# Tamnemng/TAM-GCN

Measured on AMD Instinct MI355X. Metric: skeleton clips/sec (fwd+CE+bwd+grad all-reduce+SGD step), N-UCLA 20-joint x 64-frame, higher is better.
Workload: dtype f32 (exact fp32-input MFMA v_mfma_f32_16x16x4_f32 in every GEMM, forward and backward: the reference's arithmetic); 1 GPU; N-UCLA joint stream, 256 clips/GPU x (3,64,20,1), models.ctrgcn.Model fwd+CE+bwd+grad-allreduce+SGD step, train-mode BN; global_batch=256, streams=1, parallelism=dp1, launch=hipgraph, model_streams=0, rehearsal=False, allreduce=one flat bucket after backward

## Files before the change

### include/tamgcn.h

```cpp
#ifndef TAMGCN_H
#define TAMGCN_H

#ifdef __cplusplus
extern "C" {
#endif

#define TAMGCN_VERSION 401
#define TAMGCN_MAX_SUBSETS 3
#define TAMGCN_MAX_V 32

typedef struct tamgcn_src {
    const float* x1;
    const float* x2;
    const float* coef;
    int ctot;
    int coff;
    int act;
} tamgcn_src;

int         tamgcn_version(void);
const char* tamgcn_last_error(void);
const char* tamgcn_last_kernel(void);
int         tamgcn_get_split_mode(void);
int         tamgcn_set_split_mode(int mode);

int         tamgcn_ctrgc_lds_bytes(int S, int V, int R);

typedef struct tamgcn_conv_desc {
    tamgcn_src src;
    int N, K, T_in, V;
    const float* w;
    const float* bias;
    int M, KT, dil, stride, pad;
    int wmode;
    int up;
    float* y;
    int yctot, ycoff;
    int T_out;
    int T_y;
    int ostride;
    const float* add1;
    const float* add2;
    const float* bcast;
    float bcast_scale;
    const tamgcn_src* mask;
    const float* aux;
    const float* aux_center;
    int auxctot, auxcoff;
    float* stats_part;
    int stats_ctot, stats_coff;
    const float* post_coef;
    int post_ctot, post_act;
} tamgcn_conv_desc;

int tamgcn_conv_nparts(const tamgcn_conv_desc* d);
int tamgcn_conv(const tamgcn_conv_desc* d, void* stream);

int tamgcn_conv_signmask(const tamgcn_conv_desc* d, const unsigned char* bits, int bctot, int bcoff, void* stream);

typedef struct tamgcn_wgrad_desc {
    tamgcn_src gy;
    tamgcn_src src;
    int N, M, K, T_in, T_out, V, KT, dil, stride, pad;
    float* part;
    int nsplit;
} tamgcn_wgrad_desc;
int tamgcn_wgrad_max_split(const tamgcn_wgrad_desc* d);
int tamgcn_wgrad(const tamgcn_wgrad_desc* d, void* stream);

typedef struct tamgcn_conv_pair_desc {
    int N, T, V;
    int stride;
    tamgcn_src src;
    int K, M0, M1;
    const float* w0; const float* w1;
    const float* bias0; const float* bias1;
    float* y0; int yctot0, ycoff0;
    float* y1; int yctot1, ycoff1;
    float* stats_part0; int stats_ctot0, stats_coff0;
    float* stats_part1; int stats_ctot1, stats_coff1;
} tamgcn_conv_pair_desc;
int tamgcn_conv_pair(const tamgcn_conv_pair_desc* d, void* stream);

typedef struct tamgcn_wgrad_pair_desc {
    tamgcn_src gy0, gy1, src;
    int N, M0, M1, K, T, V;
    int stride;
    float* part;
    int nsplit;
} tamgcn_wgrad_pair_desc;
int tamgcn_wgrad_pair(const tamgcn_wgrad_pair_desc* d, void* stream);

typedef struct tamgcn_reduce_desc {
    const float* part; float* out;
    int nsplit, accumulate;
    long long stride_s, count;
    float scale;
} tamgcn_reduce_desc;
int tamgcn_reduce_multi(const tamgcn_reduce_desc* descs, int n, void* stream);

int tamgcn_reduce_sum(float* part, int nsplit, long long stride_s, long long count,
                      float scale, int accumulate, float* out, void* stream);

int tamgcn_bn_fwd_finalize(const float* part, int part_ctot, int part_coff, int nparts, double count,
                           const float* gamma, const float* beta,
                           float* running_mean, float* running_var, long long* num_batches_tracked,
                           float momentum, float eps, int training,
                           float* coef, float* save, int coef_ctot, int coef_coff, int C, void* stream);

int tamgcn_coef_diff(const float* coef_d, const float* coef_y, float* out, int C, int mode, void* stream);

int tamgcn_bn_bwd_finalize(const float* part, int part_ctot, int part_coff, int nparts, double count,
                           const float* gamma, const float* save, int save_ctot, int save_coff,
                           int training, float* dgamma, float* dbeta, float* dbias_conv,
                           float* coef, int coef_ctot, int coef_coff, int C, void* stream);

typedef struct tamgcn_bn_fwd_desc {
    const float* part; int part_ctot, part_coff, nparts; double count;
    const float* gamma; const float* beta; float* running_mean; float* running_var; long long* num_batches_tracked;
    float momentum, eps; int training;
    float* coef; float* save; int coef_ctot, coef_coff, C;
} tamgcn_bn_fwd_desc;
typedef struct tamgcn_bn_bwd_desc {
    const float* part; int part_ctot, part_coff, nparts; double count;
    const float* gamma; const float* save; int save_ctot, save_coff, training;
    float* dgamma; float* dbeta; float* dbias_conv; float* coef; int coef_ctot, coef_coff, C;
} tamgcn_bn_bwd_desc;
int tamgcn_bn_fwd_finalize_multi(const tamgcn_bn_fwd_desc* descs, int n, void* stream);
int tamgcn_bn_bwd_finalize_multi(const tamgcn_bn_bwd_desc* descs, int n, void* stream);

int tamgcn_tmean(const tamgcn_src* src, int N, int C, int T, int V, float* xbar, void* stream);

typedef struct tamgcn_ctrgc_desc {
    int N, Cin, Cout, S, R, T, V;
    tamgcn_src x;
    const float* pq;
    const float* w3;
    const float* b3;
    const float* w4;
    const float* b4;
    const float* A;
    const float* alpha;
    const float* E;
} tamgcn_ctrgc_desc;

int tamgcn_ctrgc_build_e(const tamgcn_ctrgc_desc* d, float* E, void* stream);

int tamgcn_ctrgc_fwd(const tamgcn_ctrgc_desc* d, float* y, float* stats_part, float* x3_out, void* stream);

int tamgcn_ctrgc_bwd_dx3(const tamgcn_ctrgc_desc* d, const tamgcn_src* dy,
                         float* dx3, float* db3_part, void* stream);

int tamgcn_ctrgc_bwd_de_acc(const tamgcn_ctrgc_desc* d, const tamgcn_src* dy, const float* x3,
                            float* dE, void* stream);
int tamgcn_ctrgc_bwd_de_tail(const tamgcn_ctrgc_desc* d, const float* dE,
                             float* dA_part, float* dw4_part, float* db4_part,
                             float* dalpha_part, float* dpq, int groups, void* stream);

int tamgcn_ctrgc_tiled_supported(int V);
int tamgcn_ctrgc_tiled_chunks(int V);
int tamgcn_ctrgc_tiled_build_e(const tamgcn_ctrgc_desc* d, float* E, void* stream);
int tamgcn_ctrgc_tiled_agg_fwd(const tamgcn_ctrgc_desc* d, const float* x3, const float* E, float* y, float* stats_part, void* stream);
int tamgcn_ctrgc_tiled_agg_bwd(const tamgcn_ctrgc_desc* d, const tamgcn_src* dy, const float* E, float* dx3, float* db3_part, void* stream);
int tamgcn_ctrgc_tiled_de_acc(const tamgcn_ctrgc_desc* d, const tamgcn_src* dy, const float* x3, float* dE, void* stream);
int tamgcn_ctrgc_tiled_de_tail(const tamgcn_ctrgc_desc* d, const float* dE, float* dA_part, float* dw4_part, float* db4_part,
                               float* dalpha_part, float* dpq, void* stream);

int tamgcn_vgen_supported(int V);
int tamgcn_vgen_lds_bytes(int S, int V, int R);
int tamgcn_vgen_build_e(const tamgcn_ctrgc_desc* d, float* E, void* stream);
int tamgcn_vgen_agg_fwd(const tamgcn_ctrgc_desc* d, const float* x3, const float* E, float* y, float* stats_part, void* stream);
int tamgcn_vgen_agg_bwd(const tamgcn_ctrgc_desc* d, const tamgcn_src* dy, const float* E, float* dx3, float* db3_part, void* stream);
int tamgcn_vgen_de_acc(const tamgcn_ctrgc_desc* d, const tamgcn_src* dy, const float* x3, float* dE, void* stream);
int tamgcn_vgen_de_tail(const tamgcn_ctrgc_desc* d, const float* dE, float* dA_part, float* dw4_part, float* db4_part,
                        float* dalpha_part, float* dpq, int groups, void* stream);

int tamgcn_ew_nparts(int N, int C, int T, int V);

int tamgcn_gcn_tail_fwd(const tamgcn_src* y, const tamgcn_src* o, const tamgcn_src* res,
                        int N, int C, int T, int V, float* g, void* stream);
int tamgcn_gcn_tail_bwd(const float* dg, const float* g, const tamgcn_src* o, const float* o_save,
                        int N, int C, int T, int V, float* dsum, float* doz, float* part, void* stream);
int tamgcn_gcn_tail_fwd_bits(const tamgcn_src* y, const tamgcn_src* o, const tamgcn_src* res,
// ... 241 lines not shown
```

### tam_gcn_amd/_lib.py

```python
import ctypes as C
import os

_HERE = os.path.dirname(os.path.abspath(__file__))
LIB_PATH = os.path.join(_HERE, 'libtamgcn.so')

c_float_p = C.c_void_p


class Src(C.Structure):
    _fields_ = [('x1', C.c_void_p), ('x2', C.c_void_p), ('coef', C.c_void_p),
                ('ctot', C.c_int), ('coff', C.c_int), ('act', C.c_int)]


class ConvDesc(C.Structure):
    _fields_ = [('src', Src),
                ('N', C.c_int), ('K', C.c_int), ('T_in', C.c_int), ('V', C.c_int),
                ('w', C.c_void_p), ('bias', C.c_void_p),
                ('M', C.c_int), ('KT', C.c_int), ('dil', C.c_int), ('stride', C.c_int), ('pad', C.c_int),
                ('wmode', C.c_int), ('up', C.c_int),
                ('y', C.c_void_p), ('yctot', C.c_int), ('ycoff', C.c_int),
                ('T_out', C.c_int), ('T_y', C.c_int), ('ostride', C.c_int),
                ('add1', C.c_void_p), ('add2', C.c_void_p), ('bcast', C.c_void_p), ('bcast_scale', C.c_float),
                ('mask', C.POINTER(Src)),
                ('aux', C.c_void_p), ('aux_center', C.c_void_p), ('auxctot', C.c_int), ('auxcoff', C.c_int),
# ... 64 lines not shown
                ('pq', C.c_void_p), ('w3', C.c_void_p), ('b3', C.c_void_p), ('w4', C.c_void_p),
                ('b4', C.c_void_p), ('A', C.c_void_p), ('alpha', C.c_void_p), ('E', C.c_void_p)]


class F2GcnDesc(C.Structure):
    _fields_ = [(k, C.c_int) for k in ('N', 'Cin', 'Cout', 'T', 'V', 'S', 'R', 'res_mode')] + \
               [(k, C.c_void_p) for k in ('x', 'w12', 'b12', 'w4', 'b4', 'A', 'alpha', 'w3', 'b3', 'sy', 'ty', 'wd', 'bd',
                                          'E', 'sum', 'diff', 'xpart')]


class F2GemmDesc(C.Structure):
    _fields_ = [(k, C.c_int) for k in ('N', 'K', 'M', 'T', 'V', 'mode', 'relu_rows')] + \
               [(k, C.c_void_p) for k in ('x', 'w', 'b', 'add', 'out')]


class F2TcnDesc(C.Structure):
    _fields_ = [(k, C.c_int) for k in ('N', 'Cin', 'Cout', 'T', 'V', 'stride', 'Cb', 'nb', 'ks', 'res_mode')] + \
               [('dil', C.c_int * 4), ('h', C.c_void_p), ('wt', C.c_void_p * 4), ('bt', C.c_void_p * 4)] + \
               [(k, C.c_void_p) for k in ('sp', 'tp', 'x', 'wr', 'br', 'out', 'xpart')]


class F2sGcnDesc(C.Structure):
    _fields_ = [(k, C.c_int) for k in ('N', 'Cin', 'Cout', 'T', 'V', 'K')] + \
               [(k, C.c_void_p) for k in ('x', 'Ae', 'wg', 'bg', 'h')]


class F2sTcnDesc(C.Structure):
    _fields_ = [(k, C.c_int) for k in ('N', 'Cin', 'Cout', 'T', 'V', 'KT', 'stride', 'res_mode')] + \
               [(k, C.c_void_p) for k in ('h', 'wt', 'bt', 'x', 'wr', 'br', 'out')]


class F2sTcnBwdDesc(C.Structure):
    _fields_ = [(k, C.c_int) for k in ('N', 'Cout', 'T', 'V', 'KT', 'stride')] + \
               [(k, C.c_void_p) for k in ('gout', 'out', 'h', 'wtb', 'dh')]


class F2sGcnBwdDesc(C.Structure):
    _fields_ = [(k, C.c_int) for k in ('N', 'Cin', 'Cout', 'T', 'V', 'K', 'stride', 'res_mode')] + \
               [(k, C.c_void_p) for k in ('dh', 'Ae', 'wgb', 'gout', 'out', 'wrb', 'dx')]


class OptimDesc(C.Structure):
    _fields_ = [('n', C.c_longlong),
                ('p', C.c_void_p), ('g', C.c_void_p), ('s0', C.c_void_p), ('s1', C.c_void_p),
                ('lr', C.c_void_p), ('step', C.c_void_p), ('scal', C.c_void_p),
                ('mode', C.c_int), ('nesterov', C.c_int),
                ('momentum', C.c_float), ('dampening', C.c_float), ('weight_decay', C.c_float), ('eps', C.c_float),
                ('beta1', C.c_double), ('beta2', C.c_double)]


class CeDesc(C.Structure):
    _fields_ = [('logits', C.c_void_p), ('labels', C.c_void_p), ('probs', C.c_void_p), ('weight', C.c_void_p),
                ('ignore_index', C.c_longlong), ('label_smoothing', C.c_double), ('reduction', C.c_int), ('N', C.c_int), ('K', C.c_int)]


class GradGuard(C.Structure):
    _fields_ = [('max_norm', C.c_float), ('skip_nonfinite', C.c_int), ('partial', C.c_void_p), ('n_partial', C.c_int),
                ('stat', C.c_void_p), ('skipped', C.c_void_p)]


_i, _p, _d, _f, _ll = C.c_int, C.c_void_p, C.c_double, C.c_float, C.c_longlong
_SP = C.POINTER(Src)
SIGNATURES = {
    'tamgcn_version': (_i, []),
    'tamgcn_last_error': (C.c_char_p, []),
    'tamgcn_last_kernel': (C.c_char_p, []),
    'tamgcn_ctrgc_lds_bytes': (_i, [_i, _i, _i]),
    'tamgcn_get_split_mode': (_i, []),
    'tamgcn_set_split_mode': (_i, [_i]),
    'tamgcn_conv_nparts': (_i, [C.POINTER(ConvDesc)]),
    'tamgcn_conv': (_i, [C.POINTER(ConvDesc), _p]),
    'tamgcn_wgrad_max_split': (_i, [C.POINTER(WgradDesc)]),
    'tamgcn_wgrad': (_i, [C.POINTER(WgradDesc), _p]),
    'tamgcn_conv_signmask': (_i, [C.POINTER(ConvDesc), _p, _i, _i, _p]),
    'tamgcn_conv_pair': (_i, [C.POINTER(ConvPairDesc), _p]),
    'tamgcn_wgrad_pair': (_i, [C.POINTER(WgradPairDesc), _p]),
    'tamgcn_stem_stats': (_i, [_p, _p, _p, _i, _i, _i, _i, _i, _p, _p]),
    'tamgcn_stem_apply': (_i, [_p, _p, _p, _i, _i, _i, _i, _i, _p, _p]),
    'tamgcn_head_pool_fwd': (_i, [_p, _i, _i, _i, _i, _i, _p, _p]),
    'tamgcn_head_pool_bwd': (_i, [_p, _i, _i, _i, _i, _i, _p, _p]),
    'tamgcn_head_fc_fwd': (_i, [_p, _p, _p, _i, _i, _i, _p, _p]),
    'tamgcn_head_fc_bwd': (_i, [_p, _p, _p, _i, _i, _i, _p, _p, _p, _p]),
    'tamgcn_reduce_multi': (_i, [C.POINTER(ReduceDesc), _i, _p]),
    'tamgcn_reduce_sum': (_i, [_p, _i, _ll, _ll, _f, _i, _p, _p]),
    'tamgcn_bn_fwd_finalize': (_i, [_p, _i, _i, _i, _d, _p, _p, _p, _p, _p, _f, _f, _i, _p, _p, _i, _i, _i, _p]),
    'tamgcn_bn_bwd_finalize': (_i, [_p, _i, _i, _i, _d, _p, _p, _i, _i, _i, _p, _p, _p, _p, _i, _i, _i, _p]),
    'tamgcn_bn_fwd_finalize_multi': (_i, [C.POINTER(BnFwdDesc), _i, _p]),
    'tamgcn_coef_diff': (_i, [_p, _p, _p, _i, _i, _p]),
    'tamgcn_bn_bwd_finalize_multi': (_i, [C.POINTER(BnBwdDesc), _i, _p]),
    'tamgcn_tmean': (_i, [_SP, _i, _i, _i, _i, _p, _p]),
    'tamgcn_ctrgc_build_e': (_i, [C.POINTER(CtrgcDesc), _p, _p]),
    'tamgcn_ctrgc_fwd': (_i, [C.POINTER(CtrgcDesc), _p, _p, _p, _p]),
    'tamgcn_ctrgc_bwd_dx3': (_i, [C.POINTER(CtrgcDesc), _SP, _p, _p, _p]),
    'tamgcn_ctrgc_bwd_de_acc': (_i, [C.POINTER(CtrgcDesc), _SP, _p, _p, _p]),
    'tamgcn_ctrgc_bwd_de_tail': (_i, [C.POINTER(CtrgcDesc), _p, _p, _p, _p, _p, _p, _i, _p]),
    'tamgcn_ctrgc_tiled_supported': (_i, [_i]),
    'tamgcn_ctrgc_tiled_chunks': (_i, [_i]),
    'tamgcn_ctrgc_tiled_build_e': (_i, [C.POINTER(CtrgcDesc), _p, _p]),
    'tamgcn_ctrgc_tiled_agg_fwd': (_i, [C.POINTER(CtrgcDesc), _p, _p, _p, _p, _p]),
    'tamgcn_ctrgc_tiled_agg_bwd': (_i, [C.POINTER(CtrgcDesc), _SP, _p, _p, _p, _p]),
    'tamgcn_ctrgc_tiled_de_acc': (_i, [C.POINTER(CtrgcDesc), _SP, _p, _p, _p]),
    'tamgcn_ctrgc_tiled_de_tail': (_i, [C.POINTER(CtrgcDesc), _p, _p, _p, _p, _p, _p, _p]),
    'tamgcn_vgen_supported': (_i, [_i]),
    'tamgcn_vgen_lds_bytes': (_i, [_i, _i, _i]),
    'tamgcn_vgen_build_e': (_i, [C.POINTER(CtrgcDesc), _p, _p]),
    'tamgcn_vgen_agg_fwd': (_i, [C.POINTER(CtrgcDesc), _p, _p, _p, _p, _p]),
    'tamgcn_vgen_agg_bwd': (_i, [C.POINTER(CtrgcDesc), _SP, _p, _p, _p, _p]),
    'tamgcn_vgen_de_acc': (_i, [C.POINTER(CtrgcDesc), _SP, _p, _p, _p]),
    'tamgcn_vgen_de_tail': (_i, [C.POINTER(CtrgcDesc), _p, _p, _p, _p, _p, _p, _i, _p]),
    'tamgcn_ew_nparts': (_i, [_i, _i, _i, _i]),
    'tamgcn_gcn_tail_fwd': (_i, [_SP, _SP, _SP, _i, _i, _i, _i, _p, _p]),
    'tamgcn_gcn_tail_bwd': (_i, [_p, _p, _SP, _p, _i, _i, _i, _i, _p, _p, _p, _p]),
    'tamgcn_gcn_tail_fwd_bits': (_i, [_SP, _SP, _SP, _i, _i, _i, _i, _p, _p, _p]),
    'tamgcn_gcn_tail_bwd_bits': (_i, [_p, _p, _SP, _p, _i, _i, _i, _i, _p, _p, _p, _p]),
    'tamgcn_gcn_mid_bwd': (_i, [_p, _p, _p, _p, _p, _p, _i, _i, _i, _i, _p, _p, _p, _p]),
    'tamgcn_tconv_supported': (_i, [_i, _i, _i, _i, C.POINTER(C.c_int), _i, _i]),
    'tamgcn_tconv_nparts': (_i, [C.POINTER(TconvDesc), _i]),
    'tamgcn_tconv_fwd': (_i, [C.POINTER(TconvDesc), _p]),
    'tamgcn_tconv_bwd': (_i, [C.POINTER(TconvDesc), _p]),
    'tamgcn_tconv_wgrad_max_split': (_i, [C.POINTER(TconvDesc)]),
    'tamgcn_tconv_wgrad': (_i, [C.POINTER(TconvDesc), _p]),
    'tamgcn_maxpool_fwd': (_i, [_SP, _i, _i, _i, _i, _i, _p, _i, _i, _i, _p, _p]),
    'tamgcn_maxpool_post_fwd': (_i, [_SP, _i, _i, _i, _i, _i, _p, _i, _i, _i, _p, _p, _i, _p]),
    'tamgcn_maxpool_bwd': (_i, [_SP, _SP, _p, _i, _i, _i, _i, _i, _i, _p, _i, _i, _p, _p]),
    'tamgcn_add_act_fwd': (_i, [_SP, _SP, _i, _i, _i, _i, _i, _p, _p, _p, _p]),
    'tamgcn_add_act_bwd': (_i, [_p, _p, _i, _p, _p, _p, _p, _i, _i, _i, _i, _p, _p, _p]),
    'tamgcn_add_act_fwd_bits': (_i, [_SP, _SP, _i, _i, _i, _i, _p, _p, _p, _p, _p]),
    'tamgcn_add_act_bwd_bits': (_i, [_p, _p, _p, _p, _p, _p, _i, _i, _i, _i, _p, _p, _p]),
    'tamgcn_apply': (_i, [_SP, _i, _i, _i, _i, _p, _i, _i, _p]),
    'tamgcn_score_fuse': (_i, [_p, _p, _i, _i, _i, _i, _p, _p, _p, _p, _p]),
    'tamgcn_ce_fwd': (_i, [_p, _p, _i, _i, _p, _p, _p]),
    'tamgcn_ce_bwd': (_i, [_p, _p, _i, _i, _p, _p]),
    'tamgcn_ce_opts_workspace_bytes': (_ll, [C.POINTER(CeDesc)]),
    'tamgcn_ce_opts_fwd': (_i, [C.POINTER(CeDesc), _p, _p, _p, _p]),
    'tamgcn_ce_opts_bwd_rows': (_i, [_p, _p, _i, _i, _p, _p]),
    'tamgcn_eval_accumulate': (_i, [_p, _p, _p, _i, _i, _i, _p, C.POINTER(C.c_int), _i, _ll, _ll, _p, _p, _p, _p, _p]),
    'tamgcn_score_sweep': (_i, [_p, _p, C.POINTER(C.c_float), _i, _i, _i, _i, _p, _p, _p]),
    'tamgcn_stream_derive': (_i, [_p, _i, _i, _i, _i, _i, _p, _i, _p, _p]),
    'tamgcn_feeder_transform': (_i, [_p, _p, _p, _p, _p, _i, _i, _i, _i, _i, _p, _p]),
    'tamgcn_feeder_draw': (_i, [_p, _ll, _p, _i, _p, _p, _p, _i, _i, _p, _p, _p, _p, _p]),
    'tamgcn_feeder_transform_indexed': (_i, [_p, _p, _ll, _p, _p, _p, _p, _i, _i, _i, _i, _i, _p, _p]),
    'tamgcn_clip_extent': (_i, [_p, _ll, _i, _i, _i, _i, _p, _p]),
    'tamgcn_clip_draw': (_i, [_p, _ll, _p, _i, _p, _p, _i, _i, _i, _i, _i, _i, _i, _p, _p, _p, _p, _p, _p, _p, _p, _p]),
    'tamgcn_clip_transform': (_i, [_p, _ll, _p, _p, _p, _p, _i, _i, _i, _i, _i, _i, _i, _p, _p]),
    'tamgcn_clip_crop_draw': (_i, [_p, _ll, _p, _i, _p, _p, _i, _d, _d, _i, _d, _p, _p, _p, _p, _p]),
    'tamgcn_clip_resize': (_i, [_p, _ll, _p, _p, _p, _i, _i, _i, _i, _i, _i, _p, _p]),
    'tamgcn_f2_e': (_i, [C.POINTER(F2GcnDesc), _p]),
    'tamgcn_f2_gcn': (_i, [C.POINTER(F2GcnDesc), _p]),
    'tamgcn_f2_gemm': (_i, [C.POINTER(F2GemmDesc), _p]),
    'tamgcn_f2_tcn': (_i, [C.POINTER(F2TcnDesc), _p]),
    'tamgcn_f2v_e': (_i, [C.POINTER(F2GcnDesc), _p]),
    'tamgcn_f2v_gcn': (_i, [C.POINTER(F2GcnDesc), _p]),
    'tamgcn_f2v_gemm': (_i, [C.POINTER(F2GemmDesc), _p]),
    'tamgcn_f2v_tcn': (_i, [C.POINTER(F2TcnDesc), _p]),
    'tamgcn_f2g_supported': (_i, [_i]),
    'tamgcn_f2g_lds_bytes': (_i, [_i, _i, _i, _i]),
    'tamgcn_f2g_e': (_i, [C.POINTER(F2GcnDesc), _p]),
    'tamgcn_f2g_gcn': (_i, [C.POINTER(F2GcnDesc), _p]),
    'tamgcn_f2g_gemm': (_i, [C.POINTER(F2GemmDesc), _p]),
    'tamgcn_f2g_tcn': (_i, [C.POINTER(F2TcnDesc), _p]),
    'tamgcn_f2_e_grouped': (_i, [C.POINTER(F2GcnDesc), _i, _p]),
    'tamgcn_f2_gcn_grouped': (_i, [C.POINTER(F2GcnDesc), _i, _p]),
    'tamgcn_f2_gemm_grouped': (_i, [C.POINTER(F2GemmDesc), _i, _p]),
    'tamgcn_f2_tcn_grouped': (_i, [C.POINTER(F2TcnDesc), _i, _p]),
    'tamgcn_f2v_e_grouped': (_i, [C.POINTER(F2GcnDesc), _i, _p]),
    'tamgcn_f2v_gcn_grouped': (_i, [C.POINTER(F2GcnDesc), _i, _p]),
# ... 60 lines not shown
```

### tam_gcn_amd/csrc/reduce.hip

```cpp
#include "common.h"

namespace {

__global__ __launch_bounds__(256) void reduce_sum_kernel(const float* part, int nsplit, long long stride_s, long long count,
                                                         float scale, int accumulate, float* out) {
    __shared__ double red[4][64];
    const int lane = threadIdx.x & 63, w = threadIdx.x >> 6;
    const long long e = (long long)blockIdx.x * 64 + lane;
    double s = 0.0;
    if (e < count)
        for (int k = w; k < nsplit; k += 4) s += (double)part[k * stride_s + e];
    red[w][lane] = s;
    __syncthreads();
    if (w == 0 && e < count) {
        double t = (red[0][lane] + red[1][lane]) + (red[2][lane] + red[3][lane]);
        float r = (float)(t * (double)scale);
        out[e] = accumulate ? out[e] + r : r;
    }
}

}

__global__ __launch_bounds__(256) void reduce_group_kernel(float* part, int nsplit, long long stride_s, long long count) {
    __shared__ double red[4][64];
    const int lane = threadIdx.x & 63, w = threadIdx.x >> 6;
    const long long e = (long long)blockIdx.x * 64 + lane;
    const int s0 = blockIdx.y * 64, s1 = min(nsplit, s0 + 64);
    double s = 0.0;
    if (e < count)
        for (int k = s0 + w; k < s1; k += 4) s += (double)part[k * stride_s + e];
    red[w][lane] = s;
    __syncthreads();
    if (w == 0 && e < count)
        part[(long long)s0 * stride_s + e] = (float)((red[0][lane] + red[1][lane]) + (red[2][lane] + red[3][lane]));
}

constexpr int RM_MAX = 24;
struct ReduceMulti { int n; tamgcn_reduce_desc d[RM_MAX]; };

__global__ __launch_bounds__(256) void reduce_multi_kernel(const ReduceMulti md) {
    __shared__ double red[4][64];
    const tamgcn_reduce_desc& d = md.d[blockIdx.y];
    const int lane = threadIdx.x & 63, w = threadIdx.x >> 6;
    const long long e = (long long)blockIdx.x * 64 + lane;
    if ((long long)blockIdx.x * 64 >= d.count) return;
    double s = 0.0;
    if (e < d.count) {
        const float* p = d.part + e;
        int k = w;
        for (; k + 28 < d.nsplit; k += 32) {
            float a[8];
#pragma unroll
            for (int i = 0; i < 8; ++i) a[i] = p[(long long)(k + 4 * i) * d.stride_s];
            s += ((double)a[0] + (double)a[1]) + ((double)a[2] + (double)a[3]);
            s += ((double)a[4] + (double)a[5]) + ((double)a[6] + (double)a[7]);
        }
        for (; k + 12 < d.nsplit; k += 16) {
            float a0 = p[(long long)k * d.stride_s], a1 = p[(long long)(k + 4) * d.stride_s];
            float a2 = p[(long long)(k + 8) * d.stride_s], a3 = p[(long long)(k + 12) * d.stride_s];
            s += ((double)a0 + (double)a1) + ((double)a2 + (double)a3);
        }
        for (; k < d.nsplit; k += 4) s += (double)p[(long long)k * d.stride_s];
    }
    red[w][lane] = s;
    __syncthreads();
    if (w == 0 && e < d.count) {
        double t = (red[0][lane] + red[1][lane]) + (red[2][lane] + red[3][lane]);
        float r = (float)(t * (double)d.scale);
        d.out[e] = d.accumulate ? d.out[e] + r : r;
    }
}

extern "C" int tamgcn_reduce_multi(const tamgcn_reduce_desc* descs, int n, void* stream) {
    TG_CHECK(descs && n > 0, "tamgcn_reduce_multi: bad args");
    for (int i0 = 0; i0 < n; i0 += RM_MAX) {
        ReduceMulti md;
        md.n = n - i0 < RM_MAX ? n - i0 : RM_MAX;
        long long maxc = 0;
        for (int i = 0; i < md.n; ++i) {
            md.d[i] = descs[i0 + i];
            TG_CHECK(md.d[i].part && md.d[i].out && md.d[i].nsplit > 0 && md.d[i].count > 0, "tamgcn_reduce_multi: bad descriptor %d", i0 + i);
            if (md.d[i].count > maxc) maxc = md.d[i].count;
        }
        hipLaunchKernelGGL(reduce_multi_kernel, dim3((unsigned)((maxc + 63) / 64), md.n), dim3(256), 0, (hipStream_t)stream, md);
    }
    tamgcn_note_kernel("reduce_multi_kernel");
    TG_LAUNCH_CHECK("tamgcn_reduce_multi");
    return 0;
}

extern "C" int tamgcn_reduce_sum(float* part, int nsplit, long long stride_s, long long count,
                                 float scale, int accumulate, float* out, void* stream) {
    TG_CHECK(part && out && nsplit > 0 && count > 0, "tamgcn_reduce_sum: bad args");
    long long blocks = (count + 63) / 64;
    if (nsplit > 128) {
        int groups = (nsplit + 63) / 64;
        TG_CHECK(groups <= 65535, "tamgcn_reduce_sum: too many splits");
        hipLaunchKernelGGL(reduce_group_kernel, dim3((unsigned)blocks, groups), dim3(256), 0, (hipStream_t)stream,
                           part, nsplit, stride_s, count);
        nsplit = groups;
        stride_s *= 64;
    }
    hipLaunchKernelGGL(reduce_sum_kernel, dim3((unsigned)blocks), dim3(256), 0, (hipStream_t)stream,
                       part, nsplit, stride_s, count, scale, accumulate, out);
    tamgcn_note_kernel("reduce_sum_kernel");
    TG_LAUNCH_CHECK("tamgcn_reduce_sum");
    return 0;
}
```

### tam_gcn_amd/distributed.py

```python
import torch
import torch.distributed as dist


class ParamArena:

    ALIGN = 16

    def __init__(self, model):
        seen, order, starts = set(), [], []
        for m in model.modules():
            if hasattr(m, '_arena_groups'):
                for grp in m._arena_groups():
                    first = True
                    for p in grp:
                        if p.requires_grad and id(p) not in seen:
                            seen.add(id(p)); order.append(p); starts.append(first)
                            first = False
        for p in model.parameters():
            if p.requires_grad and id(p) not in seen:
                seen.add(id(p)); order.append(p); starts.append(True)
        if not order:
            raise ValueError('no trainable parameters')
        dev, dt = order[0].device, order[0].dtype
        if any(p.device != dev or p.dtype != dt for p in order):
            raise ValueError('ParamArena needs all parameters on one device with one dtype')
        self.params, self.offsets = order, []
        off = 0
        for p, st in zip(order, starts):
            if st:
                off = (off + self.ALIGN - 1) // self.ALIGN * self.ALIGN
            self.offsets.append(off)
            off += p.numel()
        self.total = (off + self.ALIGN - 1) // self.ALIGN * self.ALIGN
        self.flat = torch.zeros(self.total, device=dev, dtype=dt)
        self.epoch = 0
        with torch.no_grad():
            for p, o in zip(order, self.offsets):
                v = self.flat[o:o + p.numel()].view(p.shape)
                v.copy_(p.data)
                p.data = v
                p._tamgcn_arena = self
        ptr = self.flat.untyped_storage().data_ptr()

        def clone_views(module, state, prefix, meta):
            for k, v in list(state.items()):
                if isinstance(v, torch.Tensor) and v.untyped_storage().data_ptr() == ptr:
                    state[k] = v.clone()
        self._hook = model._register_state_dict_hook(clone_views)

    def state_version(self):
        return (self.flat._version, self.epoch)

    def touch(self):
        self.epoch += 1

    def intact(self):
        base = self.flat.data_ptr()
        return all(p.data_ptr() == base + o * p.element_size() for p, o in zip(self.params, self.offsets))

    def grad_bucket(self):
        return FlatGradBucket(self.params, offsets=self.offsets, total=self.total)


class FlatGradBucket:

    def __init__(self, params, offsets=None, total=None):
        self.params = [p for p in params if p.requires_grad]
        if not self.params:
            raise ValueError('no trainable parameters')
        dev, dt = self.params[0].device, self.params[0].dtype
        if offsets is None:
            offsets, off = [], 0
            for p in self.params:
                offsets.append(off)
                off += p.numel()
            total = off
        self.offsets = list(offsets)
        self.flat = torch.zeros(total, device=dev, dtype=dt)
        self.views = [self.flat[o:o + p.numel()].view_as(p) for p, o in zip(self.params, self.offsets)]

    def zero(self):
        for p in self.params:
            p.grad = None

    def pack(self, accumulate=False, alpha=1.0):
        if accumulate:
            pairs = [(v, p.grad) for p, v in zip(self.params, self.views) if p.grad is not None and p.grad is not v]
            if pairs:
                torch._foreach_add_([v for v, _ in pairs], [g for _, g in pairs], alpha=alpha)
            for p, v in zip(self.params, self.views):
                p.grad = v
            return self.flat
        grads = [p.grad for p in self.params]
        if any(g is None for g in grads):
            self.flat.zero_()
            pairs = [(v, g) for v, g in zip(self.views, grads) if g is not None]
            if pairs:
                torch._foreach_copy_([v for v, _ in pairs], [g for _, g in pairs])
        else:
            torch._foreach_copy_(self.views, grads)
        for p, v in zip(self.params, self.views):
            p.grad = v
        return self.flat

    def all_reduce_mean(self, group=None, local_n=None, global_n=None):
        if dist.is_available() and dist.is_initialized() and dist.get_world_size(group) > 1:
            if local_n is not None:
                if not global_n:
                    raise ValueError('all_reduce_mean: local_n needs global_n')
                self.flat.mul_(float(local_n) / float(global_n))
                dist.all_reduce(self.flat, op=dist.ReduceOp.SUM, group=group)
            else:
                dist.all_reduce(self.flat, op=dist.ReduceOp.SUM, group=group)
                self.flat.div_(dist.get_world_size(group))
        return self.flat


class SegmentedReducer:

    def __init__(self, bucket, nseg=3, group=None, comm_stream=None):
        self.bucket, self.group = bucket, group
        n = len(bucket.params)
        nseg = max(1, min(int(nseg), n))
        total = sum(p.numel() for p in bucket.params)
        bounds, acc, target = [n], 0, total / nseg
        for i in range(n - 1, 0, -1):
            acc += bucket.params[i].numel()
            if acc >= target * len(bounds) and len(bounds) < nseg:
                bounds.append(i)
        bounds.append(0)
        self.ranges = [(bounds[k + 1], bounds[k]) for k in range(len(bounds) - 1)]
        self.seg_of = {}
        for k, (lo, hi) in enumerate(self.ranges):
            for i in range(lo, hi):
                self.seg_of[id(bucket.params[i])] = k
        ends = [bucket.offsets[hi] if hi < n else bucket.flat.numel() for _, hi in self.ranges]
        self.flat_ranges = [(bucket.offsets[lo], e) for (lo, _), e in zip(self.ranges, ends)]
        self.comm = comm_stream
        self._hooks = [p.register_post_accumulate_grad_hook(self._on_grad) for p in bucket.params]
        self.begin()

    def begin(self):
        self.left = [hi - lo for lo, hi in self.ranges]
        self.sent = [False] * len(self.ranges)
        self.scale = None

    def _distributed(self):
        return dist.is_available() and dist.is_initialized() and dist.get_world_size(self.group) > 1

    def _pack(self, k):
        lo, hi = self.ranges[k]
        b = self.bucket
        pairs = [(b.views[i], b.params[i].grad) for i in range(lo, hi)]
        f0, f1 = self.flat_ranges[k]
        if any(g is None for _, g in pairs):
            b.flat[f0:f1].zero_()
        live = [(v, g) for v, g in pairs if g is not None and g.data_ptr() != v.data_ptr()]
        if live:
            torch._foreach_copy_([v for v, _ in live], [g for _, g in live])
        for i in range(lo, hi):
            b.params[i].grad = b.views[i]

    def _send(self, k, local_n=None, global_n=None):
        self._pack(k)
        self.sent[k] = True
        if not self._distributed():
            return
        f0, f1 = self.flat_ranges[k]
        seg = self.bucket.flat[f0:f1]
        if self.comm is not None and seg.is_cuda:
            self.comm.wait_stream(torch.cuda.current_stream(seg.device))
            with torch.cuda.stream(self.comm):
                dist.all_reduce(seg, op=dist.ReduceOp.SUM, group=self.group)
        else:
            dist.all_reduce(seg, op=dist.ReduceOp.SUM, group=self.group)

    def _on_grad(self, p):
        k = self.seg_of.get(id(p))
        if k is None or self.sent[k]:
            return
        self.left[k] -= 1
        if self.left[k] == 0:
            self._send(k)

    def finish(self):
        for k in range(len(self.ranges)):
            if not self.sent[k]:
                self._send(k)
        flat = self.bucket.flat
        if self.comm is not None and flat.is_cuda:
            torch.cuda.current_stream(flat.device).wait_stream(self.comm)
        if self._distributed():
            flat.div_(dist.get_world_size(self.group))
        return flat

    def remove(self):
        for h in self._hooks:
            h.remove()
        self._hooks = []


def broadcast_state(module, src=0, group=None, arena=None):
    if not (dist.is_available() and dist.is_initialized()) or dist.get_world_size(group) == 1:
        return
    rest = list(module.parameters()) + list(module.buffers())
    if arena is not None:
        if not arena.intact():
            raise ValueError('broadcast_state: the ParamArena no longer backs the parameters')
        dist.broadcast(arena.flat, src=src, group=group)
        arena.touch()
        inside = {id(p) for p in arena.params}
        rest = [t for t in rest if id(t) not in inside]
    by_type = {}
    for t in rest:
        by_type.setdefault((t.dtype, t.device), []).append(t.data)
    with torch.no_grad():
        for ts in by_type.values():
            flat = torch.cat([t.reshape(-1) for t in ts])
            dist.broadcast(flat, src=src, group=group)
            off = 0
            for t in ts:
                t.copy_(flat[off:off + t.numel()].view_as(t))
                off += t.numel()


# ... 39 lines not shown
```

### tam_gcn_amd/ops.py

```python
import ctypes as C
import os
import threading

import torch

from . import _lib
from ._lib import Src, ConvDesc, WgradDesc, CtrgcDesc, ReduceDesc, TconvDesc, TCONV_MAXB

RELU = 1


def _stream():
    return C.c_void_p(torch.cuda.current_stream().cuda_stream)


def _ptr(t):
    if t is None:
        return None
    if not (t.is_cuda and t.is_contiguous()):
        raise RuntimeError('tam_gcn_amd: expected a contiguous HIP (cuda) tensor; there is no CPU path')
    if t.dtype not in (torch.float32, torch.int64, torch.int32, torch.float64, torch.uint8):
        raise RuntimeError(f'tam_gcn_amd: unsupported dtype {t.dtype}')
    return t.data_ptr()


class S:
    __slots__ = ('x1', 'x2', 'coef', 'coff', 'act', 'ctot')

    def __init__(self, x1, x2=None, coef=None, coff=0, act=0):
        self.x1, self.x2, self.coef, self.coff, self.act = x1, x2, coef, coff, act
        self.ctot = x1.shape[1]
        if x2 is not None and x2.shape != x1.shape:
            raise RuntimeError('tam_gcn_amd: x1/x2 geometry mismatch')
        if coef is not None and tuple(coef.shape) != (3, self.ctot):
            raise RuntimeError(f'tam_gcn_amd: coef shape {tuple(coef.shape)} != (3,{self.ctot})')

    def c(self):
        return Src(_ptr(self.x1), _ptr(self.x2), _ptr(self.coef), self.ctot, self.coff, self.act)


def _lib_():
    return _lib.load()


CHUNK_ELEMS = int(os.environ.get("TAMGCN_CHUNK_ELEMS", str(2 ** 32 - 1)))


def n_chunks(N, per_clip):
    c = max(1, CHUNK_ELEMS // max(1, per_clip))
    return [(i, min(N, i + c)) for i in range(0, N, c)]


def _slice_src(src, n0, n1):
    return S(src.x1[n0:n1], None if src.x2 is None else src.x2[n0:n1], src.coef, src.coff, src.act)


SLACK = 4


def empty(*shape, like):
    n = 1
    for d_ in shape:
        n *= d_
    return torch.empty(n + SLACK, device=like.device, dtype=torch.float32)[:n].view(shape)


def empty_like(t):
    return empty(*t.shape, like=t)


def zeros_like(t):
    return empty(*t.shape, like=t).zero_()


def with_slack(t):
    if t is None or t.shape[-1] % 4 == 0:
        return t
    st = t.untyped_storage()
    if st.nbytes() - (t.storage_offset() + t.numel()) * t.element_size() >= 4 * SLACK:
        return t
    out = empty(*t.shape, like=t)
    out.copy_(t)
    return out


def conv(src, K, w, bias, M, KT=1, dil=1, stride=1, pad=0, wmode=0, up=1,
         y=None, ycoff=0, T_out=None, T_y=None, ostride=1, add1=None, add2=None,
         bcast=None, bcast_scale=0.0, mask=None, aux=None, aux_center=None, auxcoff=0, stats=False,
         post_coef=None, post_act=0, sign=None, sign_coff=0):
# ... 226 lines not shown
    return part


def tconv_wgrad_pays(V, Cb, stride):
    if V > 32:
        return True
    if V % 4:
        return Cb >= 32 or stride > 1
    return Cb >= 64


def tconv_wgrad(gy, src, Cb, KT, dils, stride):
    N, _, T_in, V = src.x1.shape
    T_out = gy.x1.shape[2]
    if V % 4:
        gy = S(with_slack(gy.x1), with_slack(gy.x2), gy.coef, gy.coff, gy.act)
        src = S(with_slack(src.x1), None, src.coef, src.coff, src.act)
    nb = len(dils)
    d = TconvDesc()
    d.src = gy.c()
    d.N, d.T_in, d.T_out, d.V, d.Cb, d.nb, d.KT, d.stride = N, T_in, T_out, V, Cb, nb, KT, stride
    for b, dl in enumerate(dils):
        d.dil[b] = int(dl)
    mc = src.c()
    d.mask = C.pointer(mc)
    lib = _lib_()
    mx = lib.tamgcn_tconv_wgrad_max_split(C.byref(d))
    if mx <= 0:
        raise RuntimeError('tamgcn_tconv_wgrad: no tiling for this shape')
    blocks = nb * (1 if Cb == 16 else (Cb // 32) ** 2)
    nsplit = max(1, min(mx, WGRAD_BLOCKS * 2 // blocks))
    part = empty(nsplit, nb, Cb, Cb, KT, like=gy.x1)
    d.y, d.yctot, d.ycoff = _ptr(part), nsplit, 0
    _lib.check(lib.tamgcn_tconv_wgrad(C.byref(d), _stream()), 'tamgcn_tconv_wgrad')
    return reduce_sum(part, nsplit, chunks=[(Cb, Cb, KT, 1)] * nb)


WGRAD_BLOCKS = int(os.environ.get('TAMGCN_WGRAD_BLOCKS', '512'))


def wgrad(gy, src, M, K, KT=1, dil=1, stride=1, pad=0, rows=None):
    N, _, T_out, V = gy.x1.shape
    T_in = src.x1.shape[2]
    per_clip = max(gy.x1.shape[1] * T_out * V, src.x1.shape[1] * T_in * V)
    chunks = n_chunks(N, per_clip) if N * per_clip > CHUNK_ELEMS else [(0, N)]
    lib = _lib_()
    descs = []
    for n0, n1 in chunks:
        g_, s_ = (gy, src) if len(chunks) == 1 else (_slice_src(gy, n0, n1), _slice_src(src, n0, n1))
        descs.append((_wgrad_desc(g_, s_, M, K, KT, dil, stride, pad), g_, s_))
    splits = [_wgrad_splits(d, len(chunks)) for d, _, _ in descs]
    nsplit = sum(splits)
    part = empty(nsplit, M, K, KT, like=gy.x1)
    off = 0
    for (d, _, _), ns in zip(descs, splits):
        d.part, d.nsplit = part.data_ptr() + 4 * off * M * K * KT, ns
        _lib.check(lib.tamgcn_wgrad(C.byref(d), _stream()), 'tamgcn_wgrad')
        off += ns
    if rows is not None:
        return reduce_sum(part, nsplit, chunks=[(m, K, KT, 1) for m in rows])
    if nsplit == 1:
        return part.view(M, K, KT, 1)
    return reduce_sum(part, nsplit).view(M, K, KT, 1)


class ReduceBatch:
    _tls = threading.local()

    @staticmethod
    def active():
        return getattr(ReduceBatch._tls, 'active', None)

    def __enter__(self):
        self.items, self.prev = [], ReduceBatch.active()
        ReduceBatch._tls.active = self
        return self

    def __exit__(self, *exc):
        ReduceBatch._tls.active = self.prev
        if self.items and exc[0] is None:
            arr = (ReduceDesc * len(self.items))()
            for i, (part, nsplit, stride, off, count, scale, acc, out) in enumerate(self.items):
                arr[i] = ReduceDesc(part.data_ptr() + 4 * off, _ptr(out), nsplit, int(acc), stride, count, scale)
            _lib.check(_lib_().tamgcn_reduce_multi(arr, len(self.items), _stream()), 'tamgcn_reduce_multi')
        self.items = []
        return False


def reduce_sum(part, nsplit, scale=1.0, out=None, accumulate=False, chunks=None, immediate=False):
    count = part.numel() // nsplit
    if chunks is not None:
        outs, off = [], 0
        flat = part.view(nsplit, count)
        for shp in chunks:
            n = 1
            for d_ in shp:
                n *= d_
            o = torch.empty(shp, device=part.device, dtype=torch.float32)
            _reduce_piece(flat, nsplit, count, off, n, scale, o)
            outs.append(o)
            off += n
        assert off == count, 'reduce_sum: chunk shapes do not cover the slab'
        return outs
    if out is None:
        out = torch.empty(part.shape[1:], device=part.device, dtype=torch.float32)
    _reduce_piece(part, nsplit, count, 0, count, scale, out, accumulate, immediate)
    return out


def _reduce_piece(part, nsplit, stride, off, count, scale, out, accumulate=False, immediate=False):
    rb = None if immediate else ReduceBatch.active()
    if rb is not None:
        rb.items.append((part, nsplit, stride, off, count, scale, accumulate, out))
        return
    src = C.c_void_p(part.data_ptr() + 4 * off)
    if nsplit > 128:
        tmp = part.view(nsplit, stride)[:, off:off + count].contiguous()
        _lib.check(_lib_().tamgcn_reduce_sum(_ptr(tmp), nsplit, count, count, scale, int(accumulate), _ptr(out), _stream()),
                   'tamgcn_reduce_sum')
        return
    _lib.check(_lib_().tamgcn_reduce_sum(src, nsplit, stride, count, scale, int(accumulate), _ptr(out), _stream()),
               'tamgcn_reduce_sum')


def coef_diff(coef_d, coef_y, mode):
    out = torch.empty_like(coef_y)
    _lib.check(_lib_().tamgcn_coef_diff(_ptr(coef_d), _ptr(coef_y), _ptr(out), coef_y.shape[1], mode, _stream()), 'tamgcn_coef_diff')
    return out


def bn_fwd_finalize(part, part_coff, count, gamma, beta, rmean, rvar, nbt, momentum, eps, training,
                    coef, save, coff, C_):
    lib = _lib_()
    if part is not None:
        pctot, nparts = part.shape[1], part.shape[2]
    else:
        pctot, nparts = 0, 0
    _lib.check(lib.tamgcn_bn_fwd_finalize(_ptr(part), pctot, part_coff, nparts, float(count),
                                          _ptr(gamma), _ptr(beta), _ptr(rmean), _ptr(rvar), _ptr(nbt),
                                          momentum, eps, int(training), _ptr(coef), _ptr(save),
                                          coef.shape[1], coff, C_, _stream()), 'tamgcn_bn_fwd_finalize')


class BNBatch:

    def __init__(self):
        self.f, self.b, self.keep = [], [], []

    def fwd(self, part, part_coff, count, gamma, beta, rmean, rvar, nbt, momentum, eps, training, coef, save, coff, C_):
        d = _lib.BnFwdDesc()
        d.part = _ptr(part)
        d.part_ctot, d.nparts = (part.shape[1], part.shape[2]) if part is not None else (0, 0)
        d.part_coff, d.count = part_coff, float(count)
        d.gamma, d.beta, d.running_mean, d.running_var, d.num_batches_tracked = _ptr(gamma), _ptr(beta), _ptr(rmean), _ptr(rvar), _ptr(nbt)
        d.momentum, d.eps, d.training = momentum, eps, int(training)
        d.coef, d.save, d.coef_ctot, d.coef_coff, d.C = _ptr(coef), _ptr(save), coef.shape[1], coff, C_
        self.f.append(d)
        self.keep += [part, coef, save]

    def bwd(self, part, part_coff, count, gamma, save, save_coff, training, dgamma, dbeta, dbias, coef, coff, C_):
        d = _lib.BnBwdDesc()
        d.part, d.part_ctot, d.part_coff, d.nparts, d.count = _ptr(part), part.shape[1], part_coff, part.shape[2], float(count)
        d.gamma, d.save, d.save_ctot, d.save_coff, d.training = _ptr(gamma), _ptr(save), save.shape[1], save_coff, int(training)
        d.dgamma, d.dbeta, d.dbias_conv = _ptr(dgamma), _ptr(dbeta), _ptr(dbias)
        d.coef, d.coef_ctot, d.coef_coff, d.C = _ptr(coef), coef.shape[1], coff, C_
        self.b.append(d)
        self.keep += [part, save, coef, dgamma, dbeta, dbias]
# ... 761 lines not shown
```

Baseline: 9404 clips/s.

## Defer weight-gradient split reductions to one batched flush into the flat grad bucket

Split-K weight-gradient reductions issued during backward are now queued on the host instead of launched one batch at a time. They are flushed at pack time as a few large queued-reduce kernels, and each destination is retargeted so the reduction writes straight into the flat all-reduce bucket view. This is meant to cut many small reduce launches and the extra foreach copy of gradients into the bucket. It also adds a deeper-unrolled reduction loop. In exchange, partial slabs stay alive longer (up to a memory cap), the host keeps queue state that must stay consistent with hipgraph capture, and a poison mode exists for debugging.

Result: no change. 9444 clips/s (median of 6 runs) (+0.4%).

```diff
diff --git a/include/tamgcn.h b/include/tamgcn.h
--- a/include/tamgcn.h
+++ b/include/tamgcn.h
@@ -99,6 +99,12 @@
 } tamgcn_reduce_desc;
 int tamgcn_reduce_multi(const tamgcn_reduce_desc* descs, int n, void* stream);
 
+int tamgcn_reduce_defer(const tamgcn_reduce_desc* descs, int n);
+int tamgcn_reduce_flush(void* stream);
+int tamgcn_reduce_pending(void);
+int tamgcn_reduce_retarget(const void* old_out, void* new_out);
+int tamgcn_reduce_discard(void);
+
 int tamgcn_reduce_sum(float* part, int nsplit, long long stride_s, long long count,
                       float scale, int accumulate, float* out, void* stream);
 
diff --git a/tam_gcn_amd/_defer.py b/tam_gcn_amd/_defer.py
--- /dev/null
+++ b/tam_gcn_amd/_defer.py
@@ -0,0 +1,157 @@
+import ctypes as C
+import math
+import os
+
+import torch
+
+from . import _lib
+
+_armed = {}
+_owner = {}
+_held = {}
+_held_bytes = {}
+_dest = {}
+
+
+def _load():
+    return _lib.load()
+
+
+def _guard(idx):
+    return torch.cuda.device(idx)
+
+
+def _stream_of(idx):
+    return torch.cuda.current_stream(idx)
+
+
+def mode():
+    v = os.environ.get('TAMGCN_DEFER_REDUCE', '1').strip().lower()
+    if v in ('0', 'off', 'false', 'no'):
+        return 'off'
+    return 'poison' if v == 'poison' else 'on'
+
+
+def max_bytes():
+    return int(os.environ.get('TAMGCN_DEFER_MAX_BYTES', str(2 << 30)))
+
+
+def _is_gpu(device):
+    return device.type == 'cuda'
+
+
+def _index(device):
+    return device.index if device.index is not None else torch.cuda.current_device()
+
+
+def armed(device):
+    return bool(_armed) and _is_gpu(device) and _index(device) in _armed
+
+
+def _clear(idx):
+    _held.pop(idx, None)
+    _held_bytes.pop(idx, None)
+    _dest.pop(idx, None)
+
+
+def _drop(idx):
+    _owner.pop(idx, None)
+    if _armed.pop(idx, None) is not None or _held.get(idx):
+        with _guard(idx):
+            _load().tamgcn_reduce_discard()
+    _clear(idx)
+
+
+def arm(device, owner=None):
+    if not _is_gpu(device):
+        return False
+    idx = _index(device)
+    _drop(idx)
+    m = mode()
+    if m == 'off':
+        return False
+    _armed[idx] = m
+    _owner[idx] = owner
+    return True
+
+
+def abandon(device, owner):
+    if _armed and _is_gpu(device):
+        idx = _index(device)
+        if idx in _armed and _owner.get(idx) == owner:
+            _drop(idx)
+
+
+def defer(device, arr, items):
+    idx = _index(device)
+    held = _held.setdefault(idx, {})
+    new = {id(it[0]): it[0] for it in items if id(it[0]) not in held}
+    nbytes = sum(p.numel() * p.element_size() for p in new.values())
+    if _held_bytes.get(idx, 0) + nbytes > max_bytes():
+        return False
+    with _guard(idx):
+        _lib.check(_load().tamgcn_reduce_defer(arr, len(items)), 'tamgcn_reduce_defer')
+    held.update(new)
+    _held_bytes[idx] = _held_bytes.get(idx, 0) + nbytes
+    dest = _dest.setdefault(idx, {})
+    poison = _armed.get(idx) == 'poison'
+    for it in items:
+        count, acc, out = it[4], it[6], it[7]
+        if not acc:
+            dest[out.data_ptr()] = count
+            if poison:
+                out.fill_(math.nan)
+    return True
+
+
+def retarget(device, pairs):
+    idx = _index(device)
+    dest = _dest.get(idx)
+    if not dest:
+        return pairs
+    rest = []
+    with _guard(idx):
+        lib = _load()
+        for v, g in pairs:
+            ptr = g.data_ptr()
+            if (dest.get(ptr) == g.numel() == v.numel() and g.dtype == v.dtype == torch.float32 and g.is_contiguous()
+                    and v.is_contiguous() and lib.tamgcn_reduce_retarget(ptr, v.data_ptr()) == 1):
+                del dest[ptr]
+                continue
+            rest.append((v, g))
+    return rest
+
+
+def flush(device):
+    if not _is_gpu(device):
+        return 0
+    idx = _index(device)
+    held = _held.get(idx)
+    if not held:
+        _clear(idx)
+        return 0
+    with _guard(idx):
+        st = _stream_of(idx)
+        for part in held.values():
+            part.record_stream(st)
+        rc = _load().tamgcn_reduce_flush(C.c_void_p(st.cuda_stream))
+    _clear(idx)
+    if rc < 0:
+        _lib.check(rc, 'tamgcn_reduce_flush')
+    return rc
+
+
+def disarm(device):
+    if not _is_gpu(device) or not (_armed or _held):
+        return 0
+    n = flush(device)
+    _armed.pop(_index(device), None)
+    _owner.pop(_index(device), None)
+    return n
+
+
+def pending(device):
+    if not _is_gpu(device):
+        return 0
+    with _guard(_index(device)):
+        return _load().tamgcn_reduce_pending()
diff --git a/tam_gcn_amd/_lib.py b/tam_gcn_amd/_lib.py
--- a/tam_gcn_amd/_lib.py
+++ b/tam_gcn_amd/_lib.py
@@ -170,6 +170,11 @@
     'tamgcn_head_fc_fwd': (_i, [_p, _p, _p, _i, _i, _i, _p, _p]),
     'tamgcn_head_fc_bwd': (_i, [_p, _p, _p, _i, _i, _i, _p, _p, _p, _p]),
     'tamgcn_reduce_multi': (_i, [C.POINTER(ReduceDesc), _i, _p]),
+    'tamgcn_reduce_defer': (_i, [C.POINTER(ReduceDesc), _i]),
+    'tamgcn_reduce_flush': (_i, [_p]),
+    'tamgcn_reduce_pending': (_i, []),
+    'tamgcn_reduce_retarget': (_i, [_p, _p]),
+    'tamgcn_reduce_discard': (_i, []),
     'tamgcn_reduce_sum': (_i, [_p, _i, _ll, _ll, _f, _i, _p, _p]),
     'tamgcn_bn_fwd_finalize': (_i, [_p, _i, _i, _i, _d, _p, _p, _p, _p, _p, _f, _f, _i, _p, _p, _i, _i, _i, _p]),
     'tamgcn_bn_bwd_finalize': (_i, [_p, _i, _i, _i, _d, _p, _p, _i, _i, _i, _p, _p, _p, _p, _i, _i, _i, _p]),
diff --git a/tam_gcn_amd/csrc/reduce.hip b/tam_gcn_amd/csrc/reduce.hip
--- a/tam_gcn_amd/csrc/reduce.hip
+++ b/tam_gcn_amd/csrc/reduce.hip
@@ -1,4 +1,7 @@
 #include "common.h"
+#include <mutex>
+#include <unordered_map>
+#include <vector>
 
 namespace {
 
@@ -38,16 +41,24 @@
 constexpr int RM_MAX = 24;
 struct ReduceMulti { int n; tamgcn_reduce_desc d[RM_MAX]; };
 
-__global__ __launch_bounds__(256) void reduce_multi_kernel(const ReduceMulti md) {
-    __shared__ double red[4][64];
-    const tamgcn_reduce_desc& d = md.d[blockIdx.y];
-    const int lane = threadIdx.x & 63, w = threadIdx.x >> 6;
-    const long long e = (long long)blockIdx.x * 64 + lane;
-    if ((long long)blockIdx.x * 64 >= d.count) return;
+template <int DEPTH>
+__device__ __forceinline__ void reduce_slabs(const tamgcn_reduce_desc& d, long long e, int lane, int w, double (*red)[64]) {
     double s = 0.0;
     if (e < d.count) {
         const float* p = d.part + e;
         int k = w;
+        if (DEPTH > 1) {
+            for (; k + 32 * DEPTH - 4 < d.nsplit; k += 32 * DEPTH) {
+                float a[8 * DEPTH];
+#pragma unroll
+                for (int i = 0; i < 8 * DEPTH; ++i) a[i] = p[(long long)(k + 4 * i) * d.stride_s];
+#pragma unroll
+                for (int j = 0; j < DEPTH; ++j) {
+                    s += ((double)a[8 * j + 0] + (double)a[8 * j + 1]) + ((double)a[8 * j + 2] + (double)a[8 * j + 3]);
+                    s += ((double)a[8 * j + 4] + (double)a[8 * j + 5]) + ((double)a[8 * j + 6] + (double)a[8 * j + 7]);
+                }
+            }
+        }
         for (; k + 28 < d.nsplit; k += 32) {
             float a[8];
 #pragma unroll
@@ -69,6 +80,30 @@
         float r = (float)(t * (double)d.scale);
         d.out[e] = d.accumulate ? d.out[e] + r : r;
     }
+}
+
+__global__ __launch_bounds__(256) void reduce_multi_kernel(const ReduceMulti md) {
+    __shared__ double red[4][64];
+    const tamgcn_reduce_desc& d = md.d[blockIdx.y];
+    const int lane = threadIdx.x & 63, w = threadIdx.x >> 6;
+    if ((long long)blockIdx.x * 64 >= d.count) return;
+    reduce_slabs<1>(d, (long long)blockIdx.x * 64 + lane, lane, w, red);
+}
+
+constexpr int RQ_MAX = 64;
+struct ReduceQueued { int n; unsigned first[RQ_MAX + 1]; tamgcn_reduce_desc d[RQ_MAX]; };
+static_assert(sizeof(ReduceQueued) <= 4096, "by-value kernel arguments");
+
+__global__ __launch_bounds__(256) void reduce_queued_kernel(const ReduceQueued qd) {
+    __shared__ double red[4][64];
+    int i = 0, hi = qd.n;
+    while (hi - i > 1) {
+        const int mid = (i + hi) >> 1;
+        if (blockIdx.x >= qd.first[mid]) i = mid; else hi = mid;
+    }
+    const tamgcn_reduce_desc& d = qd.d[i];
+    const int lane = threadIdx.x & 63, w = threadIdx.x >> 6;
+    reduce_slabs<4>(d, (long long)(blockIdx.x - qd.first[i]) * 64 + lane, lane, w, red);
 }
 
 extern "C" int tamgcn_reduce_multi(const tamgcn_reduce_desc* descs, int n, void* stream) {
@@ -87,6 +122,98 @@
     tamgcn_note_kernel("reduce_multi_kernel");
     TG_LAUNCH_CHECK("tamgcn_reduce_multi");
     return 0;
+}
+
+namespace {
+
+struct ReduceQueue {
+    std::vector<tamgcn_reduce_desc> d;
+    std::unordered_map<const void*, int> by_out;
+};
+std::mutex g_rq_mutex;
+std::unordered_map<int, ReduceQueue> g_rq;
+
+ReduceQueue& reduce_queue() {
+    int dev = 0;
+    if (hipGetDevice(&dev) != hipSuccess) { (void)hipGetLastError(); dev = 0; }
+    return g_rq[dev];
+}
+
+}
+
+extern "C" int tamgcn_reduce_defer(const tamgcn_reduce_desc* descs, int n) {
+    TG_CHECK(descs && n > 0, "tamgcn_reduce_defer: bad args");
+    for (int i = 0; i < n; ++i)
+        TG_CHECK(descs[i].part && descs[i].out && descs[i].nsplit > 0 && descs[i].count > 0 && descs[i].stride_s >= 0 &&
+                 (descs[i].count + 63) / 64 < (1ll << 31), "tamgcn_reduce_defer: bad descriptor %d", i);
+    std::lock_guard<std::mutex> lk(g_rq_mutex);
+    ReduceQueue& q = reduce_queue();
+    for (int i = 0; i < n; ++i) {
+        auto it = q.by_out.find(descs[i].out);
+        if (it == q.by_out.end()) q.by_out.emplace(descs[i].out, (int)q.d.size());
+        else it->second = -1;
+        q.d.push_back(descs[i]);
+    }
+    return 0;
+}
+
+extern "C" int tamgcn_reduce_pending(void) {
+    std::lock_guard<std::mutex> lk(g_rq_mutex);
+    return (int)reduce_queue().d.size();
+}
+
+extern "C" int tamgcn_reduce_retarget(const void* old_out, void* new_out) {
+    if (!old_out || !new_out) return 0;
+    std::lock_guard<std::mutex> lk(g_rq_mutex);
+    ReduceQueue& q = reduce_queue();
+    auto it = q.by_out.find(old_out);
+    if (it == q.by_out.end() || it->second < 0 || q.d[it->second].accumulate) return 0;
+    if (q.by_out.count(new_out)) return 0;
+    const int i = it->second;
+    q.by_out.erase(it);
+    q.by_out.emplace(new_out, i);
+    q.d[i].out = (float*)new_out;
+    return 1;
+}
+
+extern "C" int tamgcn_reduce_discard(void) {
+    std::lock_guard<std::mutex> lk(g_rq_mutex);
+    ReduceQueue& q = reduce_queue();
+    const int n = (int)q.d.size();
+    q.d.clear();
+    q.by_out.clear();
+    return n;
+}
+
+extern "C" int tamgcn_reduce_flush(void* stream) {
+    std::vector<tamgcn_reduce_desc> d;
+    {
+        std::lock_guard<std::mutex> lk(g_rq_mutex);
+        ReduceQueue& q = reduce_queue();
+        d.swap(q.d);
+        q.by_out.clear();
+    }
+    if (d.empty()) return 0;
+    int launches = 0;
+    const int n = (int)d.size();
+    for (int i0 = 0; i0 < n;) {
+        ReduceQueued qd;
+        qd.n = 0;
+        unsigned long long groups = 0;
+        while (qd.n < RQ_MAX && i0 < n) {
+            const unsigned long long g = (unsigned long long)((d[i0].count + 63) / 64);
+            if (qd.n > 0 && groups + g > 0x7fffffffull) break;
+            qd.first[qd.n] = (unsigned)groups;
+            qd.d[qd.n++] = d[i0++];
+            groups += g;
+        }
+        qd.first[qd.n] = (unsigned)groups;
+        hipLaunchKernelGGL(reduce_queued_kernel, dim3((unsigned)groups), dim3(256), 0, (hipStream_t)stream, qd);
+        ++launches;
+    }
+    tamgcn_note_kernel("reduce_queued_kernel");
+    TG_LAUNCH_CHECK("tamgcn_reduce_flush");
+    return launches;
 }
 
 extern "C" int tamgcn_reduce_sum(float* part, int nsplit, long long stride_s, long long count,
diff --git a/tam_gcn_amd/distributed.py b/tam_gcn_amd/distributed.py
--- a/tam_gcn_amd/distributed.py
+++ b/tam_gcn_amd/distributed.py
@@ -1,5 +1,7 @@
 import torch
 import torch.distributed as dist
+
+from . import _defer
 
 
 class ParamArena:
@@ -82,9 +84,21 @@
     def zero(self):
         for p in self.params:
             p.grad = None
+        _defer.arm(self.flat.device, id(self))
+
+    def __del__(self):
+        try:
+            _defer.abandon(self.flat.device, id(self))
+        except Exception:
+            pass
+
+    def flush(self):
+        _defer.disarm(self.flat.device)
 
     def pack(self, accumulate=False, alpha=1.0):
+        dev = self.flat.device
         if accumulate:
+            _defer.disarm(dev)
             pairs = [(v, p.grad) for p, v in zip(self.params, self.views) if p.grad is not None and p.grad is not v]
             if pairs:
                 torch._foreach_add_([v for v, _ in pairs], [g for _, g in pairs], alpha=alpha)
@@ -92,7 +106,14 @@
                 p.grad = v
             return self.flat
         grads = [p.grad for p in self.params]
-        if any(g is None for g in grads):
+        if _defer.armed(dev):
+            if any(g is None for g in grads):
+                self.flat.zero_()
+            pairs = _defer.retarget(dev, [(v, g) for v, g in zip(self.views, grads) if g is not None])
+            _defer.disarm(dev)
+            if pairs:
+                torch._foreach_copy_([v for v, _ in pairs], [g for _, g in pairs])
+        elif any(g is None for g in grads):
             self.flat.zero_()
             pairs = [(v, g) for v, g in zip(self.views, grads) if g is not None]
             if pairs:
@@ -141,6 +162,7 @@
         self.begin()
 
     def begin(self):
+        _defer.disarm(self.bucket.flat.device)
         self.left = [hi - lo for lo, hi in self.ranges]
         self.sent = [False] * len(self.ranges)
         self.scale = None
diff --git a/tam_gcn_amd/ops.py b/tam_gcn_amd/ops.py
--- a/tam_gcn_amd/ops.py
+++ b/tam_gcn_amd/ops.py
@@ -4,7 +4,7 @@
 
 import torch
 
-from . import _lib
+from . import _defer, _lib
 from ._lib import Src, ConvDesc, WgradDesc, CtrgcDesc, ReduceDesc, TconvDesc, TCONV_MAXB
 
 RELU = 1
@@ -397,7 +397,9 @@
             arr = (ReduceDesc * len(self.items))()
             for i, (part, nsplit, stride, off, count, scale, acc, out) in enumerate(self.items):
                 arr[i] = ReduceDesc(part.data_ptr() + 4 * off, _ptr(out), nsplit, int(acc), stride, count, scale)
-            _lib.check(_lib_().tamgcn_reduce_multi(arr, len(self.items), _stream()), 'tamgcn_reduce_multi')
+            dev = self.items[0][7].device
+            if not (_defer.armed(dev) and _defer.defer(dev, arr, self.items)):
+                _lib.check(_lib_().tamgcn_reduce_multi(arr, len(self.items), _stream()), 'tamgcn_reduce_multi')
         self.items = []
         return False
 
```
